# utiasASRL/mm_masking

Hardware: AMD Instinct MI355X
Metric: scan-pairs/s (mask-CNN + 10-iter dICP fwd+bwd) (higher is better)
Workload: dtype bf16; 1 GPU; BASELINE configs[2]: train_icp_weights step fwd+bwd, batch=32 per GPU, 10 dICP iters, point-to-plane Huber, dim=2; 400x3360 polar radar -> GO-CFAR + peaks + polar->Cartesian 640x640 -> U-Net (hand-written NHWC bf16 MFMA kernels, fp32 masters) -> dICP (fp32 points, fp64 normal equations) -> rot+trans+mask_pts loss -> Adam; batch_per_gpu=32, global_batch=32, scan_pts_pad=5120, map_pts=20000, map_pts_pad=20480, icp_iters=10, parallelism=dp1, scene_density=survey (SURVEY.md 8d: 3 500-5 000 valid scan points of 5 120)

## Files before the change

### mm_masking_amd/csrc/mmk_unet.hip

```cpp
#include <math.h>
#include <stdlib.h>

#include <algorithm>
#include <type_traits>

#include "mmk_common.h"
#include "mmk_unet_shared.h"

namespace {

using namespace mmku;

__device__ __forceinline__ unsigned cvt_pk_bf16(float lo, float hi)
{
    unsigned r;
    asm("v_cvt_pk_bf16_f32 %0, %1, %2" : "=v"(r) : "v"(lo), "v"(hi));
    return r;
}
__device__ __forceinline__ unsigned pk_relu_bf16(unsigned x)
{
    unsigned r;
    asm("v_pk_max_i16 %0, %1, 0" : "=v"(r) : "v"(x));
    return r;
}
// ... 276 lines not shown
                                const bf16x4 sv = *reinterpret_cast<const bf16x4 *>(o_src + p * o_C + cl);
#pragma unroll
                                for (int r = 0; r < 4; ++r)
                                    v[r] = lk ? v[r] * bwd_factor_leaky((float)sv[r], o_scale, a.slope)
                                              : (((float)sv[r] > 0.f) ? v[r] * o_scale : 0.f);
                            }
                            if (o_acc) {
                                const bf16x4 ov = *reinterpret_cast<const bf16x4 *>(dst);
#pragma unroll
                                for (int r = 0; r < 4; ++r) v[r] += (float)ov[r];
                            }
                            bf16x4 outv;
#pragma unroll
                            for (int r = 0; r < 4; ++r) outv[r] = (bf16)v[r];
                            *reinterpret_cast<bf16x4 *>(dst) = outv;
                        }
                    }
                }
#pragma unroll
                for (int n = 0; n < NT; ++n) acc[m][n] = (f32x4){0.f, 0.f, 0.f, 0.f};
            }
        }
        if (!has_next) break;
        __syncthreads();
        tile = ntile;
        chunk = nck;
    }
}

template <int CK, int CM, bool LK = false>
int launch_conv(const ConvArgs &a, hipStream_t st)
{
    const size_t smem = ((size_t)HT * WT * lds_pitch(CK) + (size_t)ksteps(CK) * (CM / 16) * 512) * sizeof(bf16);
    if (smem > 64 * 1024) {
        static bool attr_set[64] = {};
        int dev = 0;
        MMK_CHECK_HIP(hipGetDevice(&dev));
        if (!attr_set[dev & 63]) {
            MMK_CHECK_HIP(hipFuncSetAttribute((const void *)conv3x3_kernel<CK, CM, LK>, hipFuncAttributeMaxDynamicSharedMemorySize, (int)smem));
            attr_set[dev & 63] = true;
        }
    }
    const int tiles = ((a.W + TW - 1) / TW) * ((a.H + TH - 1) / TH);
    const int groups = (a.COUT + CM - 1) / CM;
    int per_cu = (int)std::min<size_t>(8, (160 * 1024) / smem);
    per_cu = per_cu < 1 ? 1 : per_cu;
    const int total = tiles * a.B;
    int gx = (256 * per_cu) / groups;
    gx = gx < 1 ? 1 : (gx > total ? total : gx);
    hipLaunchKernelGGL((conv3x3_kernel<CK, CM, LK>), dim3(gx, groups), dim3(CONV_THREADS), smem, st, a, total);
    MMK_LAUNCH_CHECK();
    return MMK_OK;
}


__device__ u32x4 g_zero16;
__device__ u32x4 g_zero32[2];
__device__ u32x4 g_sink32[2];
}
__device__ mmku::u32x4 mmk_sink16[8];
namespace {
#define g_sink16 mmk_sink16

__device__ __forceinline__ void unpack8(const u32x4 v, float (&f)[8])
{
#pragma unroll
    for (int j = 0; j < 4; ++j) {
        f[2 * j] = __uint_as_float(v[j] << 16);
        f[2 * j + 1] = __uint_as_float(v[j] & 0xffff0000u);
    }
}

__device__ __forceinline__ u32x4 pack8(const float (&f)[8])
{
    bf16x8 o;
#pragma unroll
    for (int j = 0; j < 8; ++j) o[j] = (bf16)f[j];
    return __builtin_bit_cast(u32x4, o);
}

__device__ __forceinline__ void lds_barrier()
{
    asm volatile("s_waitcnt lgkmcnt(0)\n\ts_barrier" ::: "memory");
}

#ifdef MMK_DEEP_STAMPS
constexpr int MMK_STAMP_STAGES = 24;
__device__ unsigned long long *g_deep_stamp_buf = nullptr;
#define MMK_STAMP(K)                                                                                          \
    do {                                                                                                      \
        if (stamp_stage < MMK_STAMP_STAGES) {                                                                 \
            const unsigned long long t_ = __builtin_amdgcn_s_memtime();                                       \
            if (lane == 0) stamp_lds[(wv * MMK_STAMP_STAGES + stamp_stage) * 8 + (K)] = t_;                    \
        }                                                                                                     \
    } while (0)
#else
#define MMK_STAMP(K) do { } while (0)
#endif

#ifndef MMK_RING_DIAG
#define MMK_RING_DIAG 0
#endif
template <int CK, int CM, int RD, bool EPI, int POOL = 0, bool C8 = false>
__global__ __launch_bounds__(CONV_THREADS) void conv3x3_ring_kernel(const ConvArgs a, int total_tiles, int tiles_per_xcd)
{
    static_assert(!(EPI && POOL), "the pooled output belongs to the forward pass (no epilogue operands)");
    static_assert(!C8 || (CM == 16 && !POOL), "C8: a single output part of exactly 8 channels");
    constexpr int NS = ksteps(CK);
    constexpr int MT = CM / 16;
    constexpr int NT = 4;
    constexpr int PK = lds_pitch(CK);
    constexpr int GPP = CK / 8;
    constexpr int NIN = HT * WT * GPP;
    constexpr int NW = NS * MT * 64;
    constexpr int RIN = (NIN + CONV_THREADS - 1) / CONV_THREADS;
    constexpr int RW = (NW + CONV_THREADS - 1) / CONV_THREADS;
    constexpr int NST = C8 ? 1 : (POOL == 2 ? 2 * MT : MT * NT + (POOL ? MT : 0));
    extern __shared__ __attribute__((aligned(16))) unsigned char smem[];
    bf16 *in_tile = reinterpret_cast<bf16 *>(smem);
    bf16 *w_lds = in_tile + 2 * HT * WT * PK;

    const int tid = threadIdx.x, lane = tid & 63, wv = tid >> 6;
    const int tiles_x = (a.W + TW - 1) / TW, tiles_y = (a.H + TH - 1) / TH;
    const int tpi = tiles_x * tiles_y;
    const int group = blockIdx.y;

    const int xcd = blockIdx.x & 7, nb = gridDim.x >> 3;
    const int t_begin = xcd * tiles_per_xcd;
    const int t_end = (t_begin + tiles_per_xcd < total_tiles) ? t_begin + tiles_per_xcd : total_tiles;
    const int first = t_begin + (blockIdx.x >> 3);
    if (first >= t_end) return;
    const int nt_blk = (t_end - first + nb - 1) / nb;
#ifdef MMK_DEEP_STAMPS
    unsigned long long *stamp_lds = reinterpret_cast<unsigned long long *>(smem + ((size_t)(2 * HT * WT * PK + NS * MT * 512) * sizeof(bf16) + 15) / 16 * 16);
    int stamp_stage = 0;
    for (int i = tid; i < 4 * MMK_STAMP_STAGES * 8; i += CONV_THREADS) stamp_lds[i] = 0ull;
    __syncthreads();
    if (tid == 0) {
        stamp_lds[6] = gridDim.x; stamp_lds[7] = (unsigned long long)nt_blk;
        stamp_lds[8 + 6] = __builtin_amdgcn_s_memtime(); stamp_lds[8 + 7] = __builtin_amdgcn_s_memrealtime();
    }
#endif

    u32x4 rin[RD][RIN];
    int g_dy[RIN], g_dx[RIN], in_off[RIN];
    bool in_x2[RIN];
#pragma unroll
    for (int i = 0; i < RIN; ++i) {
        int g = tid + i * CONV_THREADS;
        g = g < NIN ? g : NIN - 1;
        const int pix = g / GPP, c = (g % GPP) * 8;
        const int dy1 = pix / WT, dx1 = pix % WT;
        g_dy[i] = dy1 - 1;
        g_dx[i] = dx1 - 1;
        in_x2[i] = c >= a.C1;
        in_off[i] = in_x2[i] ? (dy1 * a.W + dx1) * a.C2 + (c - a.C1) : (dy1 * a.W + dx1) * a.C1 + c;
    }
    bool o_cv[MT], o_has_src[MT], o_accm[MT];
    bf16 *o_yb[MT];
    const bf16 *o_sb[MT];
    int o_C[MT], o_e0[MT], o_loff[MT][NT];
    float o_scale[MT];
#pragma unroll
    for (int m = 0; m < MT; ++m) {
        const int c0 = group * CM + m * 16 + (lane >> 4) * 4;
        const bool firstp = c0 < a.o1.C;
// ... 200 lines not shown
    const size_t smem = (((size_t)2 * HT * WT * lds_pitch(CK) + (size_t)ksteps(CK) * (CM / 16) * 512) * sizeof(bf16) + 15) / 16 * 16 +
                        (size_t)4 * MMK_STAMP_STAGES * 8 * sizeof(unsigned long long);
#else
    const size_t smem = ((size_t)2 * HT * WT * lds_pitch(CK) + (size_t)ksteps(CK) * (CM / 16) * 512) * sizeof(bf16);
#endif
    static int per_cu[64] = {};
    int dev = 0;
    MMK_CHECK_HIP(hipGetDevice(&dev));
    if (per_cu[dev & 63] == 0) {
        if (smem > 64 * 1024)
            MMK_CHECK_HIP(hipFuncSetAttribute((const void *)conv3x3_ring_kernel<CK, CM, RD, EPI, POOL, C8>,
                                               hipFuncAttributeMaxDynamicSharedMemorySize, (int)smem));
        int nblk = 0;
        MMK_CHECK_HIP(hipOccupancyMaxActiveBlocksPerMultiprocessor(&nblk, conv3x3_ring_kernel<CK, CM, RD, EPI, POOL, C8>, CONV_THREADS,
                                                                   smem));
        per_cu[dev & 63] = nblk < 1 ? 1 : (nblk > 8 ? 8 : nblk);
    }
    const int tiles = ((a.W + TW - 1) / TW) * ((a.H + TH - 1) / TH);
    const int groups = (a.COUT + CM - 1) / CM;
    const int total = tiles * a.B;
    const int per_xcd = (total + 7) / 8;
    int nb = (32 * per_cu[dev & 63]) / groups;
    nb = nb < 1 ? 1 : (nb > per_xcd ? per_xcd : nb);
    hipLaunchKernelGGL((conv3x3_ring_kernel<CK, CM, RD, EPI, POOL, C8>), dim3(8 * nb, groups), dim3(CONV_THREADS), smem, st, a, total,
                       per_xcd);
    MMK_LAUNCH_CHECK();
    return MMK_OK;
}

inline bool use_c8_epilogue()
{
    static int v = -1;
    if (v < 0) {
        const char *e = getenv("MMK_CONV_C8");
        v = (e && e[0] == '0') ? 0 : 1;
    }
    return v == 1;
}

template <int CK, int CM>
int launch_conv_ring_epi(const ConvArgs &a, hipStream_t st)
{
    constexpr int RD = CK <= 16 ? 3 : 2;
    constexpr int RDE = 2;
    const bool epi = a.o1.relu_src || a.o1.accumulate || (a.o2.C > 0 && (a.o2.relu_src || a.o2.accumulate));
    if (a.pool_y != nullptr) {
        if constexpr (CK == CM && (CK == 16 || CK == 32)) {
            if (!epi && a.o2.C == 0)
                return a.pool_arg != nullptr ? launch_conv_ring<CK, CM, RD, false, 2>(a, st) : launch_conv_ring<CK, CM, RD, false, 1>(a, st);
        }
        mmk::set_error("mmk_conv3x3: pool_y is not supported for this layer (see mmk_conv3x3_pool_fusable)");
        return MMK_ERR_ARG;
    }
    if constexpr (CM == 16) {
        if (a.COUT == 8 && a.o2.C == 0 && use_c8_epilogue())
            return epi ? launch_conv_ring<CK, CM, RDE, true, false, true>(a, st) : launch_conv_ring<CK, CM, RD, false, false, true>(a, st);
    }
    return epi ? launch_conv_ring<CK, CM, RDE, true>(a, st) : launch_conv_ring<CK, CM, RD, false>(a, st);
}


constexpr int DEEP_THREADS = 512;

template <int BM, int NT>
struct DeepCfg {
    static constexpr int WM = BM >= 128 ? 2 : 1;
    static constexpr int WN = 8 / WM;
    static constexpr int MT = BM / 16 / WM;
    static constexpr int MTB = BM / 16;
    static constexpr int TH = WN, TWD = NT * 16;
    static constexpr int HT = TH + 2, WT = TWD + 2;
    static constexpr int CK = 32, PK = 48, NS = 9, GPP = 4;
    static constexpr int NIN = HT * WT * GPP;
    static constexpr int NW = NS * MTB * 64;
    static constexpr int RIN = (NIN + DEEP_THREADS - 1) / DEEP_THREADS;
    static constexpr int RW = (NW + DEEP_THREADS - 1) / DEEP_THREADS;
    static constexpr size_t IN_BYTES = (size_t)HT * WT * PK * sizeof(bf16), W_BYTES = (size_t)NW * 8 * sizeof(bf16);
    static constexpr size_t smem_core(int wchunks) { return IN_BYTES + (size_t)wchunks * W_BYTES + BM * sizeof(float); }
#ifdef MMK_DEEP_STAMPS
    static constexpr size_t smem(int wchunks) { return (smem_core(wchunks) + 15) / 16 * 16 + (size_t)8 * MMK_STAMP_STAGES * 8 * sizeof(unsigned long long); }
#else
    static constexpr size_t smem(int wchunks) { return smem_core(wchunks); }
#endif
};

template <int BM, int NT, bool LK = false, bool SUBW = false, int ROLE = 0, bool WRES = false>
__global__ __launch_bounds__(DEEP_THREADS) void conv3x3_deep_kernel(const ConvArgs a, int total_tiles, int tiles_per_xcd)
{
    using C = DeepCfg<BM, NT>;
    constexpr int MT = C::MT, MTB = C::MTB, PK = C::PK, WT = C::WT, HT = C::HT, GPP = C::GPP;
    constexpr int NIN = C::NIN, NW = C::NW, RIN = C::RIN, RW = C::RW, NS = C::NS;
    constexpr bool R_FWD = ROLE == 1, R_BWD = ROLE == 2;
    static_assert(!(WRES && SUBW), "resident weights: the kernel's own packing only");
    extern __shared__ __attribute__((aligned(16))) unsigned char smem[];
    bf16 *in_tile = reinterpret_cast<bf16 *>(smem);
    bf16 *w_lds = in_tile + HT * WT * PK;

    const int tid = threadIdx.x, lane = tid & 63, wv = tid >> 6;
    const int wm = wv / C::WN, wn = wv % C::WN;
    const int tiles_x = (a.W + C::TWD - 1) / C::TWD, tiles_y = (a.H + C::TH - 1) / C::TH;
    const int tpi = tiles_x * tiles_y;
    const int group = blockIdx.y;
    const int nchunk = a.CIN / 32;
    const int wchunks = WRES ? nchunk : 1;

    const int xcd = blockIdx.x & 7, nb = gridDim.x >> 3;
    const int t_begin = xcd * tiles_per_xcd;
    const int t_end = (t_begin + tiles_per_xcd < total_tiles) ? t_begin + tiles_per_xcd : total_tiles;
    int tile = t_begin + (blockIdx.x >> 3);
    if (tile >= t_end) return;

    constexpr int RWL = WRES ? 0 : RW;
    u32x4 rin[RIN], rw[RW];
    int g_dy[RIN], g_dx[RIN], g_c[RIN], g_pix[RIN];
#pragma unroll
    for (int i = 0; i < RIN; ++i) {
        int g = tid + i * DEEP_THREADS;
        g = g < NIN ? g : NIN - 1;
        const int pix = g / GPP;
        g_dy[i] = pix / WT - 1;
        g_dx[i] = pix % WT - 1;
        g_c[i] = (g % GPP) * 8;
        g_pix[i] = (pix / WT) * a.W + pix % WT;
    }
    const bf16 *ld_base = nullptr;
    int ld_xc = 0, ld_ty0 = 0, ld_tx0 = 0;
    const u32x4 *ld_w = nullptr;
    int ld_moff = 0;
    auto set_stage = [&](int t, int chunk) {
        const int b = t / tpi, tr = t - b * tpi;
        const int tyi = tr / tiles_x;
        ld_tx0 = (tr - tyi * tiles_x) * C::TWD;
        ld_ty0 = tyi * C::TH;
        const int c0 = chunk * 32;
        const bool in1 = c0 < a.C1;
        const bf16 *xb = in1 ? a.x1 : a.x2;
        ld_xc = in1 ? a.C1 : a.C2;
        const int cb = in1 ? c0 : c0 - a.C1;
        const long org = ((long)b * a.H + ld_ty0 - 1) * a.W + ld_tx0 - 1;
        ld_base = xb + org * ld_xc + cb;
        if constexpr (SUBW) {
            const int pm = a.wpack_mtb, per = pm / MTB;
            ld_w = reinterpret_cast<const u32x4 *>(a.wpack + ((size_t)((group / per) * nchunk + chunk)) * NS * pm * 512);
            ld_moff = (group % per) * MTB;
        } else {
            ld_w = reinterpret_cast<const u32x4 *>(a.wpack + ((size_t)(group * nchunk + chunk)) * NW * 8);
        }
    };
    auto issue_in = [&](int i) {
        const bool ok = (unsigned)(ld_ty0 + g_dy[i]) < (unsigned)a.H && (unsigned)(ld_tx0 + g_dx[i]) < (unsigned)a.W;
        const unsigned off = (unsigned)(g_pix[i] * ld_xc + g_c[i]);
        const u32x4 *sp = ok ? reinterpret_cast<const u32x4 *>(ld_base + off) : &g_zero16;
        rin[i] = *sp;
    };
    auto issue_w = [&](int i) {
        int g = tid + i * DEEP_THREADS;
        g = g < NW ? g : NW - 1;
        if constexpr (SUBW) rw[i] = ld_w[((g / (MTB * 64)) * a.wpack_mtb + ld_moff) * 64 + g % (MTB * 64)];
        else rw[i] = ld_w[g];
    };
    auto write_in = [&]() {
#pragma unroll
        for (int i = 0; i < RIN; ++i) {
            const int g = tid + i * DEEP_THREADS;
            if (g < NIN) *reinterpret_cast<u32x4 *>(in_tile + (size_t)(g / GPP) * PK + (g % GPP) * 8) = rin[i];
        }
    };
    auto write_w = [&](int slot) {
#pragma unroll
        for (int i = 0; i < RW; ++i) {
            const int g = tid + i * DEEP_THREADS;
            if (g < NW) reinterpret_cast<u32x4 *>(w_lds + (size_t)slot * NW * 8)[g] = rw[i];
        }
    };

    const DropoutParams dp = dropout_params(a.drop_p);
    float *bias_lds = reinterpret_cast<float *>(w_lds + (size_t)wchunks * NW * 8);
    if (tid < BM) {
        int c = group * BM + tid;
        if constexpr (SUBW) {
            const int pm = a.wpack_mtb, per = pm / MTB, m_off = (group % per) * MTB;
            c = (group / per) * (pm * 16) + (m_off / 4) * 64 + 16 * (tid / (4 * MT)) + 4 * (m_off % 4) + tid % (4 * MT);
        }
        const float bz = (a.bias && c < a.COUT) ? a.bias[c] : 0.f;
        bias_lds[tid] = R_FWD ? bz * dp.inv_keep : bz;
    }
    f32x4 acc[MT][NT];
    auto reset_acc = [&]() {
#pragma unroll
        for (int m = 0; m < MT; ++m)
#pragma unroll
            for (int n = 0; n < NT; ++n) acc[m][n] = f32x4{0.f, 0.f, 0.f, 0.f};
    };
    reset_acc();

    constexpr bool lk = LK;
    const bf16 *b_base = in_tile + ((size_t)(wn * WT + (lane & 15))) * PK + 8 * (lane >> 4);
    const bf16 *a_base0 = w_lds + ((size_t)(wm * MT) * 64 + lane) * 8;

    int chunk = 0;
#ifdef MMK_DEEP_STAMPS
    unsigned long long *stamp_lds = reinterpret_cast<unsigned long long *>(smem + (C::smem_core(wchunks) + 15) / 16 * 16);
    int stamp_stage = 0;
    for (int i = tid; i < 8 * MMK_STAMP_STAGES * 8; i += DEEP_THREADS) stamp_lds[i] = 0ull;
#endif
    if constexpr (WRES) {
        for (int ck = 0; ck < nchunk; ++ck) {
            set_stage(tile, ck);
#pragma unroll
            for (int i = 0; i < RW; ++i) issue_w(i);
            write_w(ck);
        }
    }
    set_stage(tile, 0);
#pragma unroll
    for (int i = 0; i < RIN; ++i) issue_in(i);
    if constexpr (!WRES) {
#pragma unroll
        for (int i = 0; i < RW; ++i) issue_w(i);
        write_w(0);
    }
    write_in();
    __syncthreads();

    constexpr int NCH = 4 * MT;
    constexpr int LW = NCH >= 8 ? 8 : 4;
    typedef __attribute__((ext_vector_type(LW))) __bf16 bfl;
    constexpr int NP = NCH / LW;

    while (true) {
        MMK_STAMP(0);
        int ntile = tile, nck = chunk + 1;
        if (nck == nchunk) {
            nck = 0;
            ntile = tile + nb;
        }
        const bool has_next = ntile < t_end;
        set_stage(has_next ? ntile : tile, nck);
        const bf16 *a_base = a_base0 + (WRES ? (size_t)chunk * NW * 8 : (size_t)0);
        MMK_STAMP(1);
#pragma unroll
        for (int s = 0; s < NS; ++s) {
            const int ty = s / 3, tx = s % 3;
            bf16x8 bf[NT];
#pragma unroll
            for (int n = 0; n < NT; ++n)
                bf[n] = *reinterpret_cast<const bf16x8 *>(b_base + ((size_t)(ty * WT + n * 16 + tx)) * PK);
#pragma unroll
            for (int m = 0; m < MT; ++m) {
                const bf16x8 af = *reinterpret_cast<const bf16x8 *>(a_base + ((size_t)(s * MTB + m) * 64) * 8);
#pragma unroll
                for (int n = 0; n < NT; ++n) acc[m][n] = __builtin_amdgcn_mfma_f32_16x16x32_bf16(af, bf[n], acc[m][n], 0, 0, 0);
            }
#pragma unroll
            for (int j = s; j < RIN + RWL; j += NS) {
                if (j < RIN) issue_in(j);
                else issue_w(j - RIN);
            }
            __builtin_amdgcn_sched_barrier(0x38F);
        }
        MMK_STAMP(2);
        auto deliver_and_write = [&]() {
#pragma unroll
            for (int i = 0; i < RIN; ++i) asm volatile("" : "+v"(rin[i]));
#pragma unroll
            for (int i = 0; i < RWL; ++i) asm volatile("" : "+v"(rw[i]));
            MMK_STAMP(4);
            if (has_next) {
                __syncthreads();
                MMK_STAMP(5);
                write_in();
                if constexpr (!WRES) write_w(0);
            }
            MMK_STAMP(6);
        };
        if (chunk != nchunk - 1) {
            MMK_STAMP(3);
            deliver_and_write();
        } else {
            const int b = tile / tpi, tr = tile - b * tpi;
            const int tyi = tr / tiles_x;
            const int tx0 = (tr - tyi * tiles_x) * C::TWD, yy = tyi * C::TH + wn;
            int lv = lane;
            asm volatile("" : "+v"(lv));
            const int g4 = lv >> 4;
            int c0, e_bias_at;
            if constexpr (SUBW) {
                const int pm = a.wpack_mtb, per = pm / MTB, m_off = (group % per) * MTB;
                c0 = (group / per) * (pm * 16) + (m_off / 4) * 64 + 16 * g4 + 4 * (m_off % 4);
                e_bias_at = NCH * g4;
            } else {
                c0 = group * BM + wm * (16 * MT) + NCH * g4;
                e_bias_at = wm * (16 * MT) + NCH * g4;
            }
            const bool e_on = c0 < a.COUT;
            const bool firstp = c0 < a.o1.C;
            bf16 *const o_y = firstp ? a.o1.y : a.o2.y;
            const bf16 *const o_src = firstp ? a.o1.relu_src : a.o2.relu_src;
            const int o_C = firstp ? a.o1.C : a.o2.C;
            const bool e_acc = (firstp ? a.o1.accumulate : a.o2.accumulate) != 0;
            const float e_scale = firstp ? a.o1.scale : a.o2.scale;
            const int cl = firstp ? c0 : c0 - a.o1.C;
            const int e_x0 = tx0 + (lv & 15);
            const long p0 = ((long)b * a.H + yy) * a.W + e_x0;
            const unsigned e_e0 = (unsigned)p0 * (unsigned)a.COUT + (unsigned)c0 + a.hash_base;
            bf16 *const e_y0 = o_y + p0 * o_C + cl;
            const int e_step = 16 * o_C;
            const bool e_row_ok = yy < a.H;
            const bool e_src = o_src != nullptr;
            const bf16 *const e_pf0 = e_src ? o_src + p0 * o_C + cl : (e_acc ? (const bf16 *)e_y0 : nullptr);
            bfl opnd[R_BWD ? NT : 1][NP];
            auto fetch_operands = [&]() {
#pragma unroll
                for (int n = 0; n < NT; ++n) {
                    const bool okp = e_on && e_pf0 != nullptr && e_row_ok && e_x0 + n * 16 < a.W;
                    const bf16 *pp = okp ? e_pf0 + n * e_step : reinterpret_cast<const bf16 *>(g_zero32);
#pragma unroll
                    for (int k = 0; k < NP; ++k) opnd[R_BWD ? n : 0][k] = *reinterpret_cast<const bfl *>(pp + k * LW);
                }
            };
            if constexpr (R_BWD) fetch_operands();
            if (e_on) {
                if constexpr (R_FWD) {
                    float bk[NCH];
#pragma unroll
                    for (int k = 0; k < NCH; k += 4) {
                        const f32x4 t = *reinterpret_cast<const f32x4 *>(bias_lds + e_bias_at + k);
                        bk[k] = t[0]; bk[k + 1] = t[1]; bk[k + 2] = t[2]; bk[k + 3] = t[3];
                    }
                    const float kf = dp.inv_keep;
                    const int t1s = (int)dp.thr - 32768 - 1;
                    const unsigned t1 = (unsigned)(t1s < -32768 ? -32768 : t1s) & 0xffffu;
                    const unsigned thr1 = t1 | (t1 << 16);
                    const bool drop = a.drop_p > 0.f;
#pragma unroll
                    for (int n = 0; n < NT; ++n) {
                        const bool okp = e_row_ok && e_x0 + n * 16 < a.W;
                        unsigned hw[MT][2];
#pragma unroll
                        for (int m = 0; m < MT; ++m) hw[m][0] = hw[m][1] = 0x7fff7fffu;
                        if (drop) {
#pragma unroll
                            for (int m = 0; m < MT; ++m)
                                dropout_words(a.seed, e_e0 + (unsigned)n * (16u * (unsigned)a.COUT) + 4u * m, hw[m][0], hw[m][1]);
                        }
                        unsigned pk[NCH / 2];
#pragma unroll
                        for (int m = 0; m < MT; ++m)
#pragma unroll
                            for (int hlf = 0; hlf < 2; ++hlf) {
                                const float t0 = __builtin_fmaf(acc[m][n][2 * hlf], kf, bk[4 * m + 2 * hlf]);
                                const float t1f = __builtin_fmaf(acc[m][n][2 * hlf + 1], kf, bk[4 * m + 2 * hlf + 1]);
                                pk[2 * m + hlf] = pk_relu_bf16(cvt_pk_bf16(t0, t1f)) & pk_keep_mask(hw[m][hlf], thr1);
                            }
                        bf16 *const dst = okp ? e_y0 + n * e_step : reinterpret_cast<bf16 *>(g_sink32);
                        if constexpr (NCH >= 8) {
#pragma unroll
                            for (int k = 0; k < NCH / 2; k += 4)
                                *reinterpret_cast<u32x4 *>(dst + 2 * k) = (u32x4){pk[k], pk[k + 1], pk[k + 2], pk[k + 3]};
                        } else {
                            *reinterpret_cast<unsigned long long *>(dst) = ((unsigned long long)pk[1] << 32) | pk[0];
                        }
                        __builtin_amdgcn_sched_barrier(0);
                    }
                } else {
                    float bv[NCH];
                    if constexpr (!R_BWD) {
#pragma unroll
                        for (int k = 0; k < NCH; k += 4) {
                            const f32x4 t = *reinterpret_cast<const f32x4 *>(bias_lds + e_bias_at + k);
                            bv[k] = t[0]; bv[k + 1] = t[1]; bv[k + 2] = t[2]; bv[k + 3] = t[3];
                        }
                    }
                    const bool o_accf = !e_src && e_acc;
#pragma unroll
                    for (int n = 0; n < NT; ++n) {
                        const bool okp = e_row_ok && e_x0 + n * 16 < a.W;
                        float v[NCH];
#pragma unroll
                        for (int m = 0; m < MT; ++m)
#pragma unroll
                            for (int r = 0; r < 4; ++r) {
                                float t = acc[m][n][r];
                                if constexpr (!R_BWD) {
                                    t += bv[4 * m + r];
                                    if (a.relu) t = lk ? act_leaky(t, a.slope) : fmaxf(t, 0.f);
                                }
                                v[4 * m + r] = t;
                            }
                        if constexpr (!R_BWD) {
                            if (a.drop_p > 0.f) {
#pragma unroll
                                for (int m = 0; m < MT; ++m) {
                                    float sc[4];
                                    dropout_scale4(a.seed, e_e0 + (unsigned)n * (16u * (unsigned)a.COUT) + 4u * m, dp, sc);
#pragma unroll
                                    for (int r = 0; r < 4; ++r) v[4 * m + r] = lk ? drop_leaky(v[4 * m + r], sc[r]) : v[4 * m + r] * sc[r];
                                }
                            }
                        }
                        bf16 *const dst0 = e_y0 + n * e_step;
                        if constexpr (R_BWD) {
                            if (e_pf0 != nullptr && okp) {
                                if (!o_accf) {
#pragma unroll
                                    for (int k = 0; k < NCH; k += LW) {
                                        const bfl sv = opnd[n][k / LW];
#pragma unroll
                                        for (int r = 0; r < LW; ++r) v[k + r] = ((float)sv[r] > 0.f) ? v[k + r] * e_scale : 0.f;
                                    }
                                } else {
#pragma unroll
                                    for (int k = 0; k < NCH; k += LW) {
                                        const bfl ov = opnd[n][k / LW];
#pragma unroll
                                        for (int r = 0; r < LW; ++r) v[k + r] += (float)ov[r];
                                    }
                                }
                            }
                        } else {
                            if (e_src && okp) {
                                const bf16 *sp = e_pf0 + n * e_step;
#pragma unroll
                                for (int k = 0; k < NCH; k += LW) {
                                    const bfl sv = *reinterpret_cast<const bfl *>(sp + k);
#pragma unroll
                                    for (int r = 0; r < LW; ++r)
                                        v[k + r] = lk ? v[k + r] * bwd_factor_leaky((float)sv[r], e_scale, a.slope)
                                                      : (((float)sv[r] > 0.f) ? v[k + r] * e_scale : 0.f);
                                }
                            }
                            if (e_acc && okp) {
#pragma unroll
                                for (int k = 0; k < NCH; k += LW) {
                                    const bfl ov = *reinterpret_cast<const bfl *>(dst0 + k);
#pragma unroll
                                    for (int r = 0; r < LW; ++r) v[k + r] += (float)ov[r];
                                }
                            }
                        }
                        if (R_BWD || okp) {
                            bf16 *const dst = (R_BWD && !okp) ? reinterpret_cast<bf16 *>(g_sink32) : dst0;
                            if constexpr (NCH >= 8) {
#pragma unroll
                                for (int k = 0; k < NCH; k += 8) {
                                    bf16x8 o8;
#pragma unroll
                                    for (int r = 0; r < 8; ++r) o8[r] = (bf16)v[k + r];
                                    *reinterpret_cast<bf16x8 *>(dst + k) = o8;
                                }
                            } else {
                                bf16x4 o4;
#pragma unroll
                                for (int r = 0; r < 4; ++r) o4[r] = (bf16)v[r];
                                *reinterpret_cast<bf16x4 *>(dst) = o4;
                            }
                        }
                    }
                }
            }
            reset_acc();
            MMK_STAMP(3);
            deliver_and_write();
        }
        if (!has_next) break;
        __syncthreads();
        MMK_STAMP(7);
#ifdef MMK_DEEP_STAMPS
        ++stamp_stage;
#endif
        tile = ntile;
        chunk = nck;
    }
#ifdef MMK_DEEP_STAMPS
    __syncthreads();
    if (g_deep_stamp_buf != nullptr && blockIdx.y == 0 && blockIdx.x < 64)
        for (int i = tid; i < 8 * MMK_STAMP_STAGES * 8; i += DEEP_THREADS)
            g_deep_stamp_buf[(size_t)blockIdx.x * (8 * MMK_STAMP_STAGES * 8) + i] = stamp_lds[i];
#endif
}

template <int BM, int NT, bool LK = false, bool SUBW = false, int ROLE = 0, bool WRES = false>
int launch_conv_deep(const ConvArgs &a, hipStream_t st)
{
    using C = DeepCfg<BM, NT>;
    static bool attr_set[64] = {};
    int dev = 0;
    MMK_CHECK_HIP(hipGetDevice(&dev));
    if (!attr_set[dev & 63]) {
        MMK_CHECK_HIP(hipFuncSetAttribute((const void *)conv3x3_deep_kernel<BM, NT, LK, SUBW, ROLE, WRES>,
                                           hipFuncAttributeMaxDynamicSharedMemorySize, 160 * 1024));
        attr_set[dev & 63] = true;
    }
    const size_t smem = C::smem(WRES ? a.CIN / 32 : 1);
    MMK_REQUIRE(smem <= (size_t)160 * 1024, "mmk_conv3x3: %zu bytes of LDS for CIN=%d COUT=%d", smem, a.CIN, a.COUT);
    const int tiles = ((a.W + C::TWD - 1) / C::TWD) * ((a.H + C::TH - 1) / C::TH);
    const int groups = (a.COUT + BM - 1) / BM;
    const int total = tiles * a.B;
    const int per_xcd = (total + 7) / 8;
    int nb = 32 / groups;
    nb = nb < 1 ? 1 : (nb > per_xcd ? per_xcd : nb);
    hipLaunchKernelGGL((conv3x3_deep_kernel<BM, NT, LK, SUBW, ROLE, WRES>), dim3(8 * nb, groups), dim3(DEEP_THREADS), smem, st, a, total, per_xcd);
    MMK_LAUNCH_CHECK();
    return MMK_OK;
}

template <int BM, int NT>
bool deep_weights_fit(int cin) { return DeepCfg<BM, NT>::smem(cin / 32) <= (size_t)160 * 1024; }

int deep_rounds(int B, int H, int W, int cout, int BM, int NT, int *tiles_per_image)
{
    const int TH = BM >= 128 ? 4 : 8;
    const int tpi = ((W + NT * 16 - 1) / (NT * 16)) * ((H + TH - 1) / TH);
    const int groups = (cout + BM - 1) / BM;
    const int nb = std::max(1, 32 / groups), per_xcd = (B * tpi + 7) / 8;
    if (tiles_per_image) *tiles_per_image = tpi;
    return (per_xcd + nb - 1) / nb;
}

int dispatch_conv_deep_plain(const ConvArgs &a, hipStream_t st);

int dispatch_conv_deep(const ConvArgs &a, hipStream_t st)
{
    const int BM = conv_cm(a.CIN, a.COUT);
    const bool narrow = a.W <= 48;
    const int NT = narrow ? 3 : 5;
    const char *split_env = getenv("MMK_CONV_SPLIT");
    const bool split_on = !(split_env && split_env[0] == '0');
    int tpi = 0;
    const bool forward_role = a.relu != 0 && a.o1.relu_src == nullptr && a.o2.relu_src == nullptr && !a.o1.accumulate && !a.o2.accumulate;
    if (split_on && forward_role && a.slope == 0.f && (BM == 64 || BM == 128) && a.COUT % 32 == 0 && a.pool_y == nullptr && a.wpack_mtb == 0 &&
        deep_rounds(a.B, a.H, a.W, a.COUT, BM, NT, &tpi) == 2) {
        const int groups = (a.COUT + BM - 1) / BM, nb = std::max(1, 32 / groups);
        const int Bm = (8 * nb) / tpi;
        const int Bt = a.B - Bm;
        const bool under_filled = (long)a.B * tpi * groups * 10 < (long)256 * 2 * 7;
        if (Bm >= 1 && Bt >= 1 && under_filled && deep_rounds(Bm, a.H, a.W, a.COUT, BM, NT, nullptr) == 1 &&
            deep_rounds(Bt, a.H, a.W, a.COUT, 32, NT, nullptr) == 1 && (a.o1.C % 32 == 0) && (a.o2.C % 32 == 0)) {
            ConvArgs m = a;
            m.B = Bm;
            int rc = dispatch_conv_deep_plain(m, st);
            if (rc != MMK_OK) return rc;
            ConvArgs t = a;
            const size_t px = (size_t)Bm * a.H * a.W;
            t.B = Bt;
            t.x1 = a.x1 + px * a.C1;
            if (a.x2) t.x2 = a.x2 + px * a.C2;
            auto adv = [&](ConvOutPart &o) {
                if (o.y) o.y += px * o.C;
                if (o.relu_src) o.relu_src += px * o.C;
            };
            adv(t.o1);
            adv(t.o2);
            t.hash_base = a.hash_base + (unsigned)(px * a.COUT);
            t.wpack_mtb = BM / 16;
            return narrow ? launch_conv_deep<32, 3, false, true, 1>(t, st) : launch_conv_deep<32, 5, false, true, 1>(t, st);
        }
    }
    return dispatch_conv_deep_plain(a, st);
}

int dispatch_conv_deep_plain(const ConvArgs &a, hipStream_t st)
{
    const int BM = conv_cm(a.CIN, a.COUT);
    const bool narrow = a.W <= 48;
    if (a.slope > 0.f) {
#define MMK_DEEP_CASE(M) if (BM == M) return narrow ? launch_conv_deep<M, 3, true>(a, st) : launch_conv_deep<M, 5, true>(a, st)
        MMK_DEEP_CASE(16); MMK_DEEP_CASE(32); MMK_DEEP_CASE(64); MMK_DEEP_CASE(128);
#undef MMK_DEEP_CASE
    }
    const bool any_src = a.o1.relu_src != nullptr || (a.o2.C > 0 && a.o2.relu_src != nullptr);
    const bool any_acc = a.o1.accumulate != 0 || (a.o2.C > 0 && a.o2.accumulate != 0);
    const bool both1 = a.o1.relu_src != nullptr && a.o1.accumulate != 0, both2 = a.o2.C > 0 && a.o2.relu_src != nullptr && a.o2.accumulate != 0;
    const int role = (a.relu != 0 && !any_src && !any_acc) ? 1
                   : ((a.relu == 0 && a.bias == nullptr && a.drop_p == 0.f && !both1 && !both2) ? 2 : 0);
#define MMK_DEEP_CASE(M, R)                                                                                                        \
    if (BM == M && role == R) {                                                                                                    \
        if (M <= 64 && a.wpack_mtb == 0 && (narrow ? deep_weights_fit<M, 3>(a.CIN) : deep_weights_fit<M, 5>(a.CIN)))               \
            return narrow ? launch_conv_deep<M, 3, false, false, R, (M <= 64)>(a, st) : launch_conv_deep<M, 5, false, false, R, (M <= 64)>(a, st); \
        return narrow ? launch_conv_deep<M, 3, false, false, R>(a, st) : launch_conv_deep<M, 5, false, false, R>(a, st);              \
    }
    MMK_DEEP_CASE(32, 1); MMK_DEEP_CASE(64, 1); MMK_DEEP_CASE(128, 1);
    MMK_DEEP_CASE(32, 2); MMK_DEEP_CASE(64, 2); MMK_DEEP_CASE(128, 2);
#undef MMK_DEEP_CASE
#define MMK_DEEP_CASE(M) if (BM == M) return narrow ? launch_conv_deep<M, 3>(a, st) : launch_conv_deep<M, 5>(a, st)
    MMK_DEEP_CASE(16); MMK_DEEP_CASE(32); MMK_DEEP_CASE(64); MMK_DEEP_CASE(128);
#undef MMK_DEEP_CASE
    mmk::set_error("mmk_conv3x3: unsupported channel counts CIN=%d COUT=%d", a.CIN, a.COUT);
    return MMK_ERR_ARG;
}

bool pool_fusable(int cin, int cout, int B, int H, int W)
{
    const bool fits32 = (size_t)B * H * W * (size_t)std::max(cin, cout) < ((size_t)1 << 31);
    return cin == cout && (cin == 16 || cin == 32) && fits32 && H >= 2 && W >= 2;
}

int dispatch_conv(const ConvArgs &a, hipStream_t st)
{
    if (a.pool_y != nullptr && (a.slope > 0.f || !pool_fusable(a.CIN, a.COUT, a.B, a.H, a.W))) {
        mmk::set_error("mmk_conv3x3: pool_y is not supported for this layer (see mmk_conv3x3_pool_fusable)");
        return MMK_ERR_ARG;
    }
    if (conv_is_deep(a.CIN, a.COUT)) return dispatch_conv_deep(a, st);
    const int CK = conv_ck(a.CIN), CM = conv_cm(a.CIN, a.COUT);
    const bool fits32 = (size_t)a.B * a.H * a.W * (size_t)std::max(a.CIN, a.COUT) < ((size_t)1 << 31);
    if (a.slope > 0.f) {
#define MMK_CONV_CASE(K, M) if (CK == K && CM == M) return launch_conv<K, M, true>(a, st)
        MMK_CONV_CASE(8, 16); MMK_CONV_CASE(8, 32); MMK_CONV_CASE(8, 64);
        MMK_CONV_CASE(16, 16); MMK_CONV_CASE(16, 32); MMK_CONV_CASE(16, 64);
        MMK_CONV_CASE(32, 16); MMK_CONV_CASE(32, 32);
#undef MMK_CONV_CASE
    }
    if (a.CIN == CK && CM <= 32 && fits32) {
#define MMK_RING_CASE(K, M) if (CK == K && CM == M) return launch_conv_ring_epi<K, M>(a, st)
        MMK_RING_CASE(8, 16); MMK_RING_CASE(8, 32); MMK_RING_CASE(16, 16); MMK_RING_CASE(16, 32);
        MMK_RING_CASE(32, 16); MMK_RING_CASE(32, 32);
#undef MMK_RING_CASE
    }
#define MMK_CONV_CASE(K, M) if (CK == K && CM == M) return launch_conv<K, M>(a, st)
    MMK_CONV_CASE(8, 16); MMK_CONV_CASE(8, 32); MMK_CONV_CASE(8, 64);
    MMK_CONV_CASE(16, 16); MMK_CONV_CASE(16, 32); MMK_CONV_CASE(16, 64);
    MMK_CONV_CASE(32, 16); MMK_CONV_CASE(32, 32);
#undef MMK_CONV_CASE
    mmk::set_error("mmk_conv3x3: unsupported channel counts CIN=%d COUT=%d", a.CIN, a.COUT);
    return MMK_ERR_ARG;
}


typedef __attribute__((ext_vector_type(2))) int i32x2;
typedef __attribute__((ext_vector_type(4))) int i32x4;

__device__ __forceinline__ unsigned lds_addr(const void *p)
{
    return (unsigned)(size_t)(__attribute__((address_space(3))) const void *)p;
}

__device__ __forceinline__ i32x2 tr_read(unsigned addr)
{
    i32x2 v;
    asm volatile("ds_read_b64_tr_b16 %0, %1" : "=v"(v) : "v"(addr) : "memory");
    return v;
}

template <int OFF>
__device__ __forceinline__ i32x2 tr_read_o(unsigned addr)
{
    static_assert(OFF >= 0 && OFF < 65536, "ds offset field is 16 bits");
    i32x2 v;
    asm volatile("ds_read_b64_tr_b16 %0, %1 offset:%2" : "=v"(v) : "v"(addr), "n"(OFF) : "memory");
    return v;
}

__device__ __forceinline__ bf16x8 frag_from(i32x2 lo, i32x2 hi)
{
    i32x4 t = {lo.x, lo.y, hi.x, hi.y};
    return __builtin_bit_cast(bf16x8, t);
}

struct WgradArgs {
// ... 2473 lines not shown
```

Before: 3375 pairs/s.

## Stream deep conv halo and weight slices via global_load_lds DMA pipeline

Adds a DMA variant of the deep 3x3 conv kernel that loads input halos and weight slices straight into LDS with global_load_lds, skipping the register staging step. Halos are double-buffered and weights are split into three row slices that are refilled while the MFMAs run, with vmcnt waits and LDS barriers between them. The halo layout uses an XOR swizzle to avoid LDS bank conflicts. The variant is on by default for the BM=128 forward and data-gradient roles and for the split-batch tail, and can be turned off through an env var. It trades added synchronisation points and a different LDS footprint for less register pressure and better overlap of loads with compute.

New measurement: 3378 pairs/s (median of 4 runs). About the same (+0.1%).

```diff
diff --git a/mm_masking_amd/csrc/mmk_unet.hip b/mm_masking_amd/csrc/mmk_unet.hip
--- a/mm_masking_amd/csrc/mmk_unet.hip
+++ b/mm_masking_amd/csrc/mmk_unet.hip
@@ -382,6 +382,13 @@
 __device__ __forceinline__ void lds_barrier()
 {
     asm volatile("s_waitcnt lgkmcnt(0)\n\ts_barrier" ::: "memory");
+}
+
+template <int N>
+__device__ __forceinline__ void wait_vmcnt()
+{
+    static_assert(N >= 0 && N < 64, "vmcnt");
+    __builtin_amdgcn_s_waitcnt((N & 15) | ((N >> 4) << 14) | 0x0f70);
 }
 
 #ifdef MMK_DEEP_STAMPS
@@ -748,9 +755,17 @@
 #else
     static constexpr size_t smem(int wchunks) { return smem_core(wchunks); }
 #endif
+    static constexpr int HALO_G = (NIN + 63) / 64 * 64, RH = (HALO_G / 64 + 7) / 8;
+    static constexpr int SLICE_G = 3 * MTB * 64, RWS = (SLICE_G / 64 + 7) / 8;
+    static constexpr size_t dma_core() { return (size_t)2 * HALO_G * 16 + (size_t)3 * SLICE_G * 16 + BM * sizeof(float); }
+#ifdef MMK_DEEP_STAMPS
+    static constexpr size_t smem_dma() { return (dma_core() + 15) / 16 * 16 + (size_t)8 * MMK_STAMP_STAGES * 8 * sizeof(unsigned long long); }
+#else
+    static constexpr size_t smem_dma() { return dma_core(); }
+#endif
 };
 
-template <int BM, int NT, bool LK = false, bool SUBW = false, int ROLE = 0, bool WRES = false>
+template <int BM, int NT, bool LK = false, bool SUBW = false, int ROLE = 0, bool WRES = false, bool DMA = false>
 __global__ __launch_bounds__(DEEP_THREADS) void conv3x3_deep_kernel(const ConvArgs a, int total_tiles, int tiles_per_xcd)
 {
     using C = DeepCfg<BM, NT>;
@@ -758,9 +773,10 @@
     constexpr int NIN = C::NIN, NW = C::NW, RIN = C::RIN, RW = C::RW, NS = C::NS;
     constexpr bool R_FWD = ROLE == 1, R_BWD = ROLE == 2;
     static_assert(!(WRES && SUBW), "resident weights: the kernel's own packing only");
+    static_assert(!(DMA && (WRES || LK || ROLE == 0)), "DMA: the forward / data-gradient roles, weights streamed");
     extern __shared__ __attribute__((aligned(16))) unsigned char smem[];
     bf16 *in_tile = reinterpret_cast<bf16 *>(smem);
-    bf16 *w_lds = in_tile + HT * WT * PK;
+    bf16 *w_lds = in_tile + (DMA ? 2 * C::HALO_G * 8 : HT * WT * PK);
 
     const int tid = threadIdx.x, lane = tid & 63, wv = tid >> 6;
     const int wm = wv / C::WN, wn = wv % C::WN;
@@ -841,7 +857,7 @@
     };
 
     const DropoutParams dp = dropout_params(a.drop_p);
-    float *bias_lds = reinterpret_cast<float *>(w_lds + (size_t)wchunks * NW * 8);
+    float *bias_lds = reinterpret_cast<float *>(w_lds + (DMA ? (size_t)3 * C::SLICE_G * 8 : (size_t)wchunks * NW * 8));
     if (tid < BM) {
         int c = group * BM + tid;
         if constexpr (SUBW) {
@@ -866,28 +882,82 @@
 
     int chunk = 0;
 #ifdef MMK_DEEP_STAMPS
-    unsigned long long *stamp_lds = reinterpret_cast<unsigned long long *>(smem + (C::smem_core(wchunks) + 15) / 16 * 16);
+    unsigned long long *stamp_lds = reinterpret_cast<unsigned long long *>(smem + ((DMA ? C::dma_core() : C::smem_core(wchunks)) + 15) / 16 * 16);
     int stamp_stage = 0;
     for (int i = tid; i < 8 * MMK_STAMP_STAGES * 8; i += DEEP_THREADS) stamp_lds[i] = 0ull;
 #endif
-    if constexpr (WRES) {
-        for (int ck = 0; ck < nchunk; ++ck) {
-            set_stage(tile, ck);
+    constexpr int HG = C::HALO_G, NJH = HG / 64, RH = C::RH;
+    constexpr int SG = C::SLICE_G, NJW = SG / 64, RWS = C::RWS;
+    constexpr unsigned W_OFF = 2u * HG * 16;
+    const int wvu = DMA ? __builtin_amdgcn_readfirstlane(wv) : 0;
+    int h_dy[RH], h_dx[RH], h_c[RH], h_pix[RH];
+    if constexpr (DMA) {
+#pragma unroll
+        for (int r = 0; r < RH; ++r) {
+            const int c = (r * 8 + wvu < NJH) ? r * 8 + wvu : NJH - 1;
+            const int G = c * 64 + lane, p = G >> 2;
+            const int q = (G & 3) ^ ((p >> 1) & 2);
+            const bool pad = p >= HT * WT;
+            h_dy[r] = pad ? -(1 << 24) : p / WT - 1;
+            h_dx[r] = p % WT - 1;
+            h_c[r] = q * 8;
+            h_pix[r] = (p / WT) * a.W + p % WT;
+        }
+    }
+    auto dma16 = [&](const void *src, unsigned lds_byte) {
+        __builtin_amdgcn_global_load_lds((const __attribute__((address_space(1))) void *)src,
+                                         (__attribute__((address_space(3))) void *)(smem + lds_byte), 16, 0, 0);
+    };
+    auto issue_halo = [&](int buf) {
+#pragma unroll
+        for (int r = 0; r < RH; ++r) {
+            const int c = (r * 8 + wvu < NJH) ? r * 8 + wvu : NJH - 1;
+            const bool ok = (unsigned)(ld_ty0 + h_dy[r]) < (unsigned)a.H && (unsigned)(ld_tx0 + h_dx[r]) < (unsigned)a.W;
+            const unsigned off = (unsigned)(h_pix[r] * ld_xc + h_c[r]);
+            dma16(ok ? (const void *)(ld_base + off) : (const void *)&g_zero16, (unsigned)buf * (HG * 16) + c * 1024);
+        }
+    };
+    auto issue_slice = [&](int slot) {
+#pragma unroll
+        for (int r = 0; r < RWS; ++r) {
+            const int c = (r * 8 + wvu < NJW) ? r * 8 + wvu : NJW - 1;
+            const int g = c * 64 + lane;
+            const u32x4 *src;
+            if constexpr (SUBW) src = ld_w + ((3 * slot + g / (MTB * 64)) * a.wpack_mtb + ld_moff) * 64 + g % (MTB * 64);
+            else src = ld_w + 3 * slot * (MTB * 64) + g;
+            dma16(src, W_OFF + (unsigned)slot * (SG * 16) + c * 1024);
+        }
+    };
+    const unsigned b_lane = (unsigned)((wn * WT + (lane & 15)) * 64 + 16 * (lane >> 4));
+    int hb = 0;
+
+    if constexpr (DMA) {
+        set_stage(tile, 0);
+        issue_slice(0);
+        issue_slice(1);
+        issue_halo(0);
+        wait_vmcnt<0>();
+        __syncthreads();
+    } else {
+        if constexpr (WRES) {
+            for (int ck = 0; ck < nchunk; ++ck) {
+                set_stage(tile, ck);
+#pragma unroll
+                for (int i = 0; i < RW; ++i) issue_w(i);
+                write_w(ck);
+            }
+        }
+        set_stage(tile, 0);
+#pragma unroll
+        for (int i = 0; i < RIN; ++i) issue_in(i);
+        if constexpr (!WRES) {
 #pragma unroll
             for (int i = 0; i < RW; ++i) issue_w(i);
-            write_w(ck);
-        }
-    }
-    set_stage(tile, 0);
-#pragma unroll
-    for (int i = 0; i < RIN; ++i) issue_in(i);
-    if constexpr (!WRES) {
-#pragma unroll
-        for (int i = 0; i < RW; ++i) issue_w(i);
-        write_w(0);
-    }
-    write_in();
-    __syncthreads();
+            write_w(0);
+        }
+        write_in();
+        __syncthreads();
+    }
 
     constexpr int NCH = 4 * MT;
     constexpr int LW = NCH >= 8 ? 8 : 4;
@@ -902,28 +972,64 @@
             ntile = tile + nb;
         }
         const bool has_next = ntile < t_end;
-        set_stage(has_next ? ntile : tile, nck);
-        const bf16 *a_base = a_base0 + (WRES ? (size_t)chunk * NW * 8 : (size_t)0);
-        MMK_STAMP(1);
-#pragma unroll
-        for (int s = 0; s < NS; ++s) {
-            const int ty = s / 3, tx = s % 3;
-            bf16x8 bf[NT];
-#pragma unroll
-            for (int n = 0; n < NT; ++n)
-                bf[n] = *reinterpret_cast<const bf16x8 *>(b_base + ((size_t)(ty * WT + n * 16 + tx)) * PK);
-#pragma unroll
-            for (int m = 0; m < MT; ++m) {
-                const bf16x8 af = *reinterpret_cast<const bf16x8 *>(a_base + ((size_t)(s * MTB + m) * 64) * 8);
-#pragma unroll
-                for (int n = 0; n < NT; ++n) acc[m][n] = __builtin_amdgcn_mfma_f32_16x16x32_bf16(af, bf[n], acc[m][n], 0, 0, 0);
-            }
-#pragma unroll
-            for (int j = s; j < RIN + RWL; j += NS) {
-                if (j < RIN) issue_in(j);
-                else issue_w(j - RIN);
-            }
-            __builtin_amdgcn_sched_barrier(0x38F);
+        if constexpr (DMA) {
+            const bool defer = R_BWD && chunk == nchunk - 1;
+            const unsigned hbase = (unsigned)hb * (HG * 16);
+#pragma unroll
+            for (int i = 0; i < 3; ++i) {
+                if (i == 0) {
+                    issue_slice(2);
+                    set_stage(has_next ? ntile : tile, nck);
+                    issue_halo(hb ^ 1);
+                } else if (i == 1 || !defer) {
+                    issue_slice(i - 1);
+                }
+#pragma unroll
+                for (int s = 3 * i; s < 3 * i + 3; ++s) {
+                    const int ty = s / 3, tx = s % 3;
+                    bf16x8 bf[NT];
+#pragma unroll
+                    for (int n = 0; n < NT; ++n) {
+                        const unsigned x = b_lane + (unsigned)((ty * WT + n * 16 + tx) * 64);
+                        bf[n] = *reinterpret_cast<const bf16x8 *>(smem + hbase + (x ^ ((x >> 3) & 32u)));
+                    }
+#pragma unroll
+                    for (int m = 0; m < MT; ++m) {
+                        const bf16x8 af = *reinterpret_cast<const bf16x8 *>(a_base0 + ((size_t)(s * MTB + m) * 64) * 8);
+#pragma unroll
+                        for (int n = 0; n < NT; ++n) acc[m][n] = __builtin_amdgcn_mfma_f32_16x16x32_bf16(af, bf[n], acc[m][n], 0, 0, 0);
+                    }
+                }
+                if (i < 2) {
+                    wait_vmcnt<RH + RWS>();
+                    lds_barrier();
+                    MMK_STAMP(1 + 3 * i);
+                }
+            }
+        } else {
+            set_stage(has_next ? ntile : tile, nck);
+            const bf16 *a_base = a_base0 + (WRES ? (size_t)chunk * NW * 8 : (size_t)0);
+            MMK_STAMP(1);
+#pragma unroll
+            for (int s = 0; s < NS; ++s) {
+                const int ty = s / 3, tx = s % 3;
+                bf16x8 bf[NT];
+#pragma unroll
+                for (int n = 0; n < NT; ++n)
+                    bf[n] = *reinterpret_cast<const bf16x8 *>(b_base + ((size_t)(ty * WT + n * 16 + tx)) * PK);
+#pragma unroll
+                for (int m = 0; m < MT; ++m) {
+                    const bf16x8 af = *reinterpret_cast<const bf16x8 *>(a_base + ((size_t)(s * MTB + m) * 64) * 8);
+#pragma unroll
+                    for (int n = 0; n < NT; ++n) acc[m][n] = __builtin_amdgcn_mfma_f32_16x16x32_bf16(af, bf[n], acc[m][n], 0, 0, 0);
+                }
+#pragma unroll
+                for (int j = s; j < RIN + RWL; j += NS) {
+                    if (j < RIN) issue_in(j);
+                    else issue_w(j - RIN);
+                }
+                __builtin_amdgcn_sched_barrier(0x38F);
+            }
         }
         MMK_STAMP(2);
         auto deliver_and_write = [&]() {
@@ -942,8 +1048,13 @@
         };
         if (chunk != nchunk - 1) {
             MMK_STAMP(3);
-            deliver_and_write();
+            if constexpr (DMA) wait_vmcnt<RWS>();
+            else deliver_and_write();
         } else {
+            if constexpr (DMA) {
+                if constexpr (R_BWD) wait_vmcnt<0>();
+                else wait_vmcnt<RWS>();
+            }
             const int b = tile / tpi, tr = tile - b * tpi;
             const int tyi = tr / tiles_x;
             const int tx0 = (tr - tyi * tiles_x) * C::TWD, yy = tyi * C::TH + wn;
@@ -985,7 +1096,15 @@
                     for (int k = 0; k < NP; ++k) opnd[R_BWD ? n : 0][k] = *reinterpret_cast<const bfl *>(pp + k * LW);
                 }
             };
-            if constexpr (R_BWD) fetch_operands();
+            if constexpr (R_BWD) {
+                fetch_operands();
+                if constexpr (DMA) {
+#pragma unroll
+                    for (int n = 0; n < NT; ++n)
+#pragma unroll
+                        for (int k = 0; k < NP; ++k) asm volatile("" ::"v"(opnd[n][k]));
+                }
+            }
             if (e_on) {
                 if constexpr (R_FWD) {
                     float bk[NCH];
@@ -1127,10 +1246,19 @@
             }
             reset_acc();
             MMK_STAMP(3);
-            deliver_and_write();
+            if constexpr (DMA) {
+                if constexpr (R_BWD) issue_slice(1);
+            } else {
+                deliver_and_write();
+            }
         }
         if (!has_next) break;
-        __syncthreads();
+        if constexpr (DMA) {
+            lds_barrier();
+            hb ^= 1;
+        } else {
+            __syncthreads();
+        }
         MMK_STAMP(7);
 #ifdef MMK_DEEP_STAMPS
         ++stamp_stage;
@@ -1138,6 +1266,7 @@
         tile = ntile;
         chunk = nck;
     }
+    if constexpr (DMA) wait_vmcnt<0>();
 #ifdef MMK_DEEP_STAMPS
     __syncthreads();
     if (g_deep_stamp_buf != nullptr && blockIdx.y == 0 && blockIdx.x < 64)
@@ -1146,7 +1275,7 @@
 #endif
 }
 
-template <int BM, int NT, bool LK = false, bool SUBW = false, int ROLE = 0, bool WRES = false>
+template <int BM, int NT, bool LK = false, bool SUBW = false, int ROLE = 0, bool WRES = false, bool DMA = false>
 int launch_conv_deep(const ConvArgs &a, hipStream_t st)
 {
     using C = DeepCfg<BM, NT>;
@@ -1154,11 +1283,12 @@
     int dev = 0;
     MMK_CHECK_HIP(hipGetDevice(&dev));
     if (!attr_set[dev & 63]) {
-        MMK_CHECK_HIP(hipFuncSetAttribute((const void *)conv3x3_deep_kernel<BM, NT, LK, SUBW, ROLE, WRES>,
+        MMK_CHECK_HIP(hipFuncSetAttribute((const void *)conv3x3_deep_kernel<BM, NT, LK, SUBW, ROLE, WRES, DMA>,
                                            hipFuncAttributeMaxDynamicSharedMemorySize, 160 * 1024));
         attr_set[dev & 63] = true;
     }
-    const size_t smem = C::smem(WRES ? a.CIN / 32 : 1);
+    static_assert(!DMA || C::smem_dma() <= (size_t)160 * 1024, "DMA pipeline: LDS budget");
+    const size_t smem = DMA ? C::smem_dma() : C::smem(WRES ? a.CIN / 32 : 1);
     MMK_REQUIRE(smem <= (size_t)160 * 1024, "mmk_conv3x3: %zu bytes of LDS for CIN=%d COUT=%d", smem, a.CIN, a.COUT);
     const int tiles = ((a.W + C::TWD - 1) / C::TWD) * ((a.H + C::TH - 1) / C::TH);
     const int groups = (a.COUT + BM - 1) / BM;
@@ -1166,7 +1296,7 @@
     const int per_xcd = (total + 7) / 8;
     int nb = 32 / groups;
     nb = nb < 1 ? 1 : (nb > per_xcd ? per_xcd : nb);
-    hipLaunchKernelGGL((conv3x3_deep_kernel<BM, NT, LK, SUBW, ROLE, WRES>), dim3(8 * nb, groups), dim3(DEEP_THREADS), smem, st, a, total, per_xcd);
+    hipLaunchKernelGGL((conv3x3_deep_kernel<BM, NT, LK, SUBW, ROLE, WRES, DMA>), dim3(8 * nb, groups), dim3(DEEP_THREADS), smem, st, a, total, per_xcd);
     MMK_LAUNCH_CHECK();
     return MMK_OK;
 }
@@ -1185,6 +1315,12 @@
 }
 
 int dispatch_conv_deep_plain(const ConvArgs &a, hipStream_t st);
+
+bool deep_dma_on()
+{
+    const char *e = getenv("MMK_DEEP_DMA");
+    return !(e && e[0] == '0');
+}
 
 int dispatch_conv_deep(const ConvArgs &a, hipStream_t st)
 {
@@ -1220,6 +1356,8 @@
             adv(t.o2);
             t.hash_base = a.hash_base + (unsigned)(px * a.COUT);
             t.wpack_mtb = BM / 16;
+            if (deep_dma_on())
+                return narrow ? launch_conv_deep<32, 3, false, true, 1, false, true>(t, st) : launch_conv_deep<32, 5, false, true, 1, false, true>(t, st);
             return narrow ? launch_conv_deep<32, 3, false, true, 1>(t, st) : launch_conv_deep<32, 5, false, true, 1>(t, st);
         }
     }
@@ -1240,8 +1378,10 @@
     const bool both1 = a.o1.relu_src != nullptr && a.o1.accumulate != 0, both2 = a.o2.C > 0 && a.o2.relu_src != nullptr && a.o2.accumulate != 0;
     const int role = (a.relu != 0 && !any_src && !any_acc) ? 1
                    : ((a.relu == 0 && a.bias == nullptr && a.drop_p == 0.f && !both1 && !both2) ? 2 : 0);
+    const bool dma = deep_dma_on();
 #define MMK_DEEP_CASE(M, R)                                                                                                        \
     if (BM == M && role == R) {                                                                                                    \
+        if (M == 128 && dma) return narrow ? launch_conv_deep<128, 3, false, false, R, false, true>(a, st) : launch_conv_deep<128, 5, false, false, R, false, true>(a, st); \
         if (M <= 64 && a.wpack_mtb == 0 && (narrow ? deep_weights_fit<M, 3>(a.CIN) : deep_weights_fit<M, 5>(a.CIN)))               \
             return narrow ? launch_conv_deep<M, 3, false, false, R, (M <= 64)>(a, st) : launch_conv_deep<M, 5, false, false, R, (M <= 64)>(a, st); \
         return narrow ? launch_conv_deep<M, 3, false, false, R>(a, st) : launch_conv_deep<M, 5, false, false, R>(a, st);              \
```
